# allenai/embodied-clip

Hardware: AMD Instinct MI355X
Metric: env-frames/sec (CLIP encode + policy fwd/bwd + PPO update) (higher is better)
Workload: dtype bf16

## Files before the change

embodied_clip_amd/csrc/conv_igemm.hip:

```cpp
#include <stdlib.h>

#include <algorithm>
#include <type_traits>
#include <utility>

#include "common.h"

thread_local int ec_tls_conv8_min_tiles = EC_CONV8_MIN_TILES_DEFAULT;

namespace {

inline int ec_tools_ablate() {
#ifdef EC_TOOLS
    static const int v = [] { const char* e = getenv("EC_CONV_ABLATE"); return e ? atoi(e) : 0; }();
    return v;
#else
    return 0;
#endif
}

constexpr int BK = 64;
constexpr int ROW_BYTES = BK * 2;

struct ConvArgs {
// ... 35 lines not shown

__device__ __forceinline__ float ec_relu(float x) { return __builtin_amdgcn_fmed3f(x, 0.f, __builtin_inff()); }
template <int ACT, bool RES, bool POOL, int FM, int FN, int PITCH>
__device__ __forceinline__ void epi_stage(const f32x16_t (&acc)[FM][FN], unsigned char* smem, const float* bias_n0,
                                          int row0, int col0, int lane) {
    const int frow = lane & 31, fhalf = lane >> 5;
#pragma unroll
    for (int j = 0; j < FN; ++j) {
        constexpr bool BIAS_UP_FRONT = !(RES && FM * FN <= 4);
        float4 bvj[4];
        if constexpr (BIAS_UP_FRONT) {
#pragma unroll
            for (int g = 0; g < 4; ++g)
                bvj[g] = bias_n0 ? *reinterpret_cast<const float4*>(bias_n0 + col0 + j * 32 + 8 * g + 4 * fhalf)
                                 : make_float4(0.f, 0.f, 0.f, 0.f);
        }
#pragma unroll
        for (int g = 0; g < 4; ++g) {
            if constexpr (!BIAS_UP_FRONT)
                bvj[g] = bias_n0 ? *reinterpret_cast<const float4*>(bias_n0 + col0 + j * 32 + 8 * g + 4 * fhalf)
                                 : make_float4(0.f, 0.f, 0.f, 0.f);
            const int lcol = col0 + j * 32 + 8 * g + 4 * fhalf;
            uint2 rr[FM];
            if constexpr (RES) {
#pragma unroll
                for (int i = 0; i < FM; ++i)
                    rr[i] = *reinterpret_cast<const uint2*>(smem + (row0 + i * 32 + frow) * PITCH + lcol * 2);
            }
#pragma unroll
            for (int i = 0; i < FM; ++i) {
                const int lrow_px = row0 + i * 32 + frow;
                float v0 = acc[i][j][4 * g + 0] + bvj[g].x, v1 = acc[i][j][4 * g + 1] + bvj[g].y;
                float v2 = acc[i][j][4 * g + 2] + bvj[g].z, v3 = acc[i][j][4 * g + 3] + bvj[g].w;
                if constexpr (POOL) {
                    v0 = ec_relu(v0); v1 = ec_relu(v1); v2 = ec_relu(v2); v3 = ec_relu(v3);
                    v0 += dpp_quad_xor1(v0); v1 += dpp_quad_xor1(v1); v2 += dpp_quad_xor1(v2); v3 += dpp_quad_xor1(v3);
                    v0 += dpp_quad_xor2(v0); v1 += dpp_quad_xor2(v1); v2 += dpp_quad_xor2(v2); v3 += dpp_quad_xor2(v3);
                    if ((lane & 3) == 0) {
                        uint2 o;
                        o.x = ec_pack2(0.25f * v0, 0.25f * v1);
                        o.y = ec_pack2(0.25f * v2, 0.25f * v3);
                        *reinterpret_cast<uint2*>(smem + (lrow_px >> 2) * PITCH + lcol * 2) = o;
                    }
                } else {
                    if constexpr (RES) {
                        v0 += ec_lo(rr[i].x); v1 += ec_hi(rr[i].x); v2 += ec_lo(rr[i].y); v3 += ec_hi(rr[i].y);
                    }
                    if constexpr (ACT == EC_ACT_RELU) {
                        v0 = ec_relu(v0); v1 = ec_relu(v1); v2 = ec_relu(v2); v3 = ec_relu(v3);
                    } else if constexpr (ACT == EC_ACT_QUICKGELU) {
                        v0 *= __builtin_amdgcn_rcpf(1.f + __expf(-1.702f * v0)); v1 *= __builtin_amdgcn_rcpf(1.f + __expf(-1.702f * v1));
                        v2 *= __builtin_amdgcn_rcpf(1.f + __expf(-1.702f * v2)); v3 *= __builtin_amdgcn_rcpf(1.f + __expf(-1.702f * v3));
                    }
                    uint2 o;
                    o.x = ec_pack2(v0, v1);
                    o.y = ec_pack2(v2, v3);
                    *reinterpret_cast<uint2*>(smem + lrow_px * PITCH + lcol * 2) = o;
                }
            }
        }
    }
}
template <bool POOL, bool RES_ONLY, int FM, int FN, int PITCH>
__device__ __forceinline__ void epi_stage_dispatch(const f32x16_t (&acc)[FM][FN], unsigned char* smem, const float* bias_n0,
                                                   int row0, int col0, int lane, int act, bool has_res) {
    if constexpr (POOL) {
        epi_stage<EC_ACT_RELU, false, true, FM, FN, PITCH>(acc, smem, bias_n0, row0, col0, lane);
    } else if constexpr (RES_ONLY) {
        if (act == EC_ACT_RELU) epi_stage<EC_ACT_RELU, true, false, FM, FN, PITCH>(acc, smem, bias_n0, row0, col0, lane);
        else epi_stage<EC_ACT_NONE, true, false, FM, FN, PITCH>(acc, smem, bias_n0, row0, col0, lane);
    } else {
        if (act == EC_ACT_RELU) {
            if (has_res) epi_stage<EC_ACT_RELU, true, false, FM, FN, PITCH>(acc, smem, bias_n0, row0, col0, lane);
            else epi_stage<EC_ACT_RELU, false, false, FM, FN, PITCH>(acc, smem, bias_n0, row0, col0, lane);
        } else if (act == EC_ACT_QUICKGELU) {
            epi_stage<EC_ACT_QUICKGELU, false, false, FM, FN, PITCH>(acc, smem, bias_n0, row0, col0, lane);
        } else {
            if (has_res) epi_stage<EC_ACT_NONE, true, false, FM, FN, PITCH>(acc, smem, bias_n0, row0, col0, lane);
            else epi_stage<EC_ACT_NONE, false, false, FM, FN, PITCH>(acc, smem, bias_n0, row0, col0, lane);
        }
    }
}

template <int ACT, int FM, int FN, int PITCH>
__device__ __forceinline__ void epi_stage_ln(const f32x16_t (&acc)[FM][FN], unsigned char* smem, const float* s_n0, const float* c_n0,
                                             const float2* rowab, int row0, int col0, int lane) {
    const int frow = lane & 31, fhalf = lane >> 5;
    float2 ab[FM];
#pragma unroll
    for (int i = 0; i < FM; ++i) ab[i] = rowab[row0 + i * 32 + frow];
#pragma unroll
    for (int j = 0; j < FN; ++j) {
        float4 sv[4], cv[4];
#pragma unroll
        for (int g = 0; g < 4; ++g) {
            sv[g] = *reinterpret_cast<const float4*>(s_n0 + col0 + j * 32 + 8 * g + 4 * fhalf);
            cv[g] = *reinterpret_cast<const float4*>(c_n0 + col0 + j * 32 + 8 * g + 4 * fhalf);
        }
#pragma unroll
        for (int g = 0; g < 4; ++g) {
            const int lcol = col0 + j * 32 + 8 * g + 4 * fhalf;
#pragma unroll
            for (int i = 0; i < FM; ++i) {
                const int lrow_px = row0 + i * 32 + frow;
                float v0 = fmaf(ab[i].x, acc[i][j][4 * g + 0], fmaf(ab[i].y, sv[g].x, cv[g].x));
                float v1 = fmaf(ab[i].x, acc[i][j][4 * g + 1], fmaf(ab[i].y, sv[g].y, cv[g].y));
                float v2 = fmaf(ab[i].x, acc[i][j][4 * g + 2], fmaf(ab[i].y, sv[g].z, cv[g].z));
                float v3 = fmaf(ab[i].x, acc[i][j][4 * g + 3], fmaf(ab[i].y, sv[g].w, cv[g].w));
                if constexpr (ACT == EC_ACT_QUICKGELU) {
                    v0 *= __builtin_amdgcn_rcpf(1.f + __expf(-1.702f * v0)); v1 *= __builtin_amdgcn_rcpf(1.f + __expf(-1.702f * v1));
                    v2 *= __builtin_amdgcn_rcpf(1.f + __expf(-1.702f * v2)); v3 *= __builtin_amdgcn_rcpf(1.f + __expf(-1.702f * v3));
                } else if constexpr (ACT == EC_ACT_RELU) {
                    v0 = ec_relu(v0); v1 = ec_relu(v1); v2 = ec_relu(v2); v3 = ec_relu(v3);
                }
                uint2 o;
                o.x = ec_pack2(v0, v1);
                o.y = ec_pack2(v2, v3);
                *reinterpret_cast<uint2*>(smem + lrow_px * PITCH + lcol * 2) = o;
            }
        }
    }
}

template <int R>
struct FragRing { u32x4_t f[R]; };
template <int I, int R, class AddrFn>
__device__ __forceinline__ void fr_issue(FragRing<R>& ring, AddrFn& addr) {
    asm volatile("ds_read_b128 %0, %1" : "=v"(ring.f[I % R]) : "v"(addr(std::integral_constant<int, I>{})));
}
template <int I, int R>
__device__ __forceinline__ void fr_tie(FragRing<R>& ring) { asm volatile("" : "+v"(ring.f[I % R])); }
template <int K, int NK, int G, int R, class AddrFn, class MmaFn>
__device__ __forceinline__ void fr_step(FragRing<R>& ring, AddrFn& addr, MmaFn& mma) {
    if constexpr (K < NK) {
        if constexpr (K + 1 < NK) {
            [&]<int... Q>(std::integer_sequence<int, Q...>) { (fr_issue<(K + 1) * G + Q, R>(ring, addr), ...); }
            (std::make_integer_sequence<int, G>{});
        }
        constexpr int after = (K + 1 < NK) ? G : 0;
        static_assert(G <= 15, "lgkmcnt is a 4-bit counter");
        asm volatile("s_waitcnt lgkmcnt(%0)" : : "n"(after));
        [&]<int... Q>(std::integer_sequence<int, Q...>) { (fr_tie<K * G + Q, R>(ring), ...); }(std::make_integer_sequence<int, G>{});
        mma(std::integral_constant<int, K>{}, ring);
        fr_step<K + 1, NK, G, R>(ring, addr, mma);
    }
}

template <int BM, int BN, int WM, int WN, int KS, bool POOL, bool PF, int MV, int NS, bool ILV = false, bool S2 = false>
__global__ __launch_bounds__(WM * WN * 64, (BM > 192) ? 2 : ((WM * WN == 8) ? 4 : (NS >= 3 ? 2 : 3))) void conv_igemm_kernel(ConvArgs p) {
    constexpr int TM = BM / WM, TN = BN / WN;
    constexpr int FM = TM / 32, FN = TN / 32;
    constexpr int NT = WM * WN * 64;
    constexpr int LR = NT / 8;
    constexpr int A_IT = BM / LR, B_IT = BN / LR;
    constexpr int A_BYTES = BM * ROW_BYTES, B_BYTES = BN * ROW_BYTES;
    static_assert(WM * WN == 4 || WM * WN == 8, "4 or 8 waves");
    static_assert(BM % LR == 0 && BN % LR == 0, "loader geometry");
    extern __shared__ __attribute__((aligned(16))) unsigned char smem[];

    const int tid = threadIdx.x;
    const int lane = tid & 63;
    const int wave = tid >> 6;
    const int wm = wave / WN, wn = wave % WN;

    const unsigned grid = gridDim.x;
    const unsigned lb = ec_xcd_remap(blockIdx.x, grid);
    static_assert(!ILV || (NS >= 3 && !PF && FM + FN <= 4), "interleaved pieces: ring mode with the inline-asm fragment stream");
    const int nvt = p.ntiles;
    int vt = (int)lb;
    if (vt >= nvt) return;
    int tile = vt;
    static_assert(MV <= BM && (MV == BM || !POOL), "padded tiles: non-pooled only");
    int m0 = (tile / p.ntn) * MV;
    int n0 = (tile % p.ntn) * BN;


    const int chunk = (tid & 7) ^ ((tid >> 4) & 7);
    const int lrow = tid >> 3;
    unsigned a_off[A_IT];
    unsigned a_msk[A_IT];
    unsigned b_off[B_IT];
    auto decode = [&]() {
#pragma unroll
        for (int i = 0; i < A_IT; ++i) {
            const int m = m0 + lrow + LR * i;
            int pix, y = 0, x = 0;
            if (POOL) {
                const int q = m >> 2, s2 = m & 3;
                const int Hp = p.H >> 1, Wp = p.W >> 1;
                const int b = q / (Hp * Wp);
                const int r2 = q - b * (Hp * Wp);
                const int yp = r2 / Wp;
                y = 2 * yp + (s2 >> 1);
                x = 2 * (r2 - yp * Wp) + (s2 & 1);
                pix = (b * p.H + y) * p.W + x;
            } else if (S2) {
                static_assert(!S2 || !POOL, "stride-2 instances have no fused pool");
                const int Ho = p.H >> 1, Wo = p.W >> 1;
                const int b = m / (Ho * Wo);
                const int r2 = m - b * (Ho * Wo);
                const int yo = r2 / Wo;
                y = 2 * yo;
// ... 201 lines not shown
                if (!(p.ablate & 2)) compute(cur);
                __syncthreads();
            }
        }
        }
        vt += (int)grid;
        const bool has_next = vt < nvt;
        if (has_next) {
            tile = vt;
            m0 = (tile / p.ntn) * MV;
            n0 = (tile % p.ntn) * BN;
            decode();
        }
        if (!(p.ablate & 8)) {
    if (has_res) {
        if (PREFETCH) {
#pragma unroll
            for (int i = 0; i < (PREFETCH ? NPASS : 1); ++i)
                *reinterpret_cast<uint4*>(smem + (i * RPP + srow) * PITCH + schunk * 16) = rres[i];
        } else {
#pragma unroll
            for (int i = 0; i < NPASS; ++i) {
                const int row = i * RPP + srow;
                uint4 v = make_uint4(0, 0, 0, 0);
#if defined(__HIP_DEVICE_COMPILE__)
                const unsigned off = (MV == BM || row < MV) ? ((unsigned)(orow0 + row) * (unsigned)p.Cout + (unsigned)(e_n0 + schunk * 8)) * 2u : 0xFFFFFFF0u;
                v = __builtin_bit_cast(uint4, __builtin_amdgcn_raw_buffer_load_b128(rs_res, (int)off, 0, 0));
#endif
                *reinterpret_cast<uint4*>(smem + row * PITCH + schunk * 16) = v;
            }
        }
        __syncthreads();
    }
    epi_stage_dispatch<POOL, PF, FM, FN, PITCH>(acc, smem, p.bias ? p.bias + e_n0 : nullptr, wm * TM, wn * TN, lane, p.act, has_res);
    __syncthreads();
#pragma unroll
    for (int r0 = 0; r0 < OUT_ROWS; r0 += RPP) {
        const int row = r0 + srow;
        if (orow0 + row < Mout && (MV == BM || row < MV))
            *reinterpret_cast<uint4*>(p.out + (long)(orow0 + row) * p.ldo + e_n0 + schunk * 8) =
                *reinterpret_cast<const uint4*>(smem + row * PITCH + schunk * 16);
    }
        }
        if (!has_next) break;
        __syncthreads();
    }
}

template <int BM, int BN, int WM, int WN, int KS, bool POOL, bool PF = false, int MV = BM, int NS = 0, bool ILV = false, bool S2 = false>
int launch(const ConvArgs& a, hipStream_t s) {
    ConvArgs p = a;
    p.ntn = a.Cout / BN;
    const int ntm = (a.M + MV - 1) / MV;
    p.ntiles = ntm * p.ntn;
    const size_t lds_max = 2 * (size_t)(BM + BN) * ROW_BYTES;
    const size_t epi = (size_t)(POOL ? BM / 4 : BM) * (BN * 2 + 16);
    p.nbuf = (BM * BN >= 256 * 256) ? 2 : 1;
    p.ablate = ec_tools_ablate();
    size_t lds = (size_t)(NS >= 3 ? NS : p.nbuf) * (BM + BN) * ROW_BYTES;
    if (lds < epi) lds = epi;
    auto kern = conv_igemm_kernel<BM, BN, WM, WN, KS, POOL, PF, MV, NS, ILV, S2>;
    static std::atomic<uint64_t> attr_done{0};
    if (auto attr_g_ = ec_attr_needed(attr_done)) {
        const size_t want = NS >= 3 ? lds : (lds_max > epi ? lds_max : epi);
        (void)hipFuncSetAttribute(reinterpret_cast<const void*>(kern), hipFuncAttributeMaxDynamicSharedMemorySize, (int)want);
    }
    const int wg_cap = 768;
    const int ring_per_cu = NS >= 3 ? (int)std::min<size_t>(2, (160 * 1024) / lds) : 0;
    const int cap = NS >= 3 ? 256 * ring_per_cu : ((BM * BN >= 256 * 256) ? 256 : wg_cap);
    const int nwg = p.ntiles < cap ? p.ntiles : cap;
    hipLaunchKernelGGL(kern, dim3((unsigned)nwg), dim3(WM * WN * 64), lds, s, p);
    EC_CHECK_LAUNCH();
    return EC_OK;
}


__device__ unsigned long long ec_dbg_stamps[2 * 1024];

template <int BN, int KS, bool POOL, int ABL, bool X3 = false, bool S2 = false, int BM = 256, int XP = 3>
__global__ __launch_bounds__(512, 2) void conv_igemm8_kernel(ConvArgs p) {
    static_assert(BM == 256 || (BM == 192 && BN == 128 && !POOL && !X3), "tile heights: 256; 192 for 128-wide 1x1 / 3x3 tiles");
    constexpr int WN = (BN >= 256 || BM == 192) ? 4 : 2, WMW = 8 / WN;
    constexpr int TM = BM / WMW, TN = BN / WN;
    constexpr int FM = TM / 32, FN = TN / 32;
    constexpr int NT = 512, LR = NT / 8;
    constexpr int A_IT = BM / LR, B_IT = BN / LR;
    constexpr int A_BYTES = BM * ROW_BYTES, B_BYTES = BN * ROW_BYTES, STAGE = A_BYTES + B_BYTES;
    static_assert(FN >= 1 && B_IT >= 1, "BN must be 128 or 256");
    constexpr bool LS = (ABL & 512) != 0 && BN == 128;
    extern __shared__ __attribute__((aligned(16))) unsigned char smem[];

    const unsigned long long t_entry = (ABL & 32) ? __builtin_amdgcn_s_memtime() : 0ull;
    const int tid = threadIdx.x;
    const int lane = tid & 63;
    const int wave = __builtin_amdgcn_readfirstlane(tid >> 6);
    const int wm = wave / WN, wn = wave % WN;
    const int grp = wave >> 2;

    const int tile = (int)ec_xcd_remap(blockIdx.x, gridDim.x);
    if (tile >= p.ntiles) return;
    const int m0 = (tile / p.ntn) * BM;
    const int n0 = (tile % p.ntn) * BN;

    constexpr bool LNOK = (KS == 1) && !POOL && !X3 && !S2;
    if constexpr (LNOK) {
        if (p.ln_stats && tid < BM) {
            float2 ab = make_float2(0.f, 0.f);
            const int row = m0 + tid;
            if (row < p.M) {
                const float4* rec = reinterpret_cast<const float4*>(p.ln_stats) + (size_t)row * p.ln_np;
                float4 r[8];
                float S = 0.f, Nn = 0.f;
#pragma unroll
                for (int q = 0; q < 8; ++q)
                    if (q < p.ln_np) { r[q] = rec[q]; S += r[q].x; Nn += r[q].z; }
                const float mean = S / Nn;
                float M2 = 0.f;
#pragma unroll
                for (int q = 0; q < 8; ++q)
                    if (q < p.ln_np) { const float d = r[q].x / r[q].z - mean; M2 += r[q].y + r[q].z * d * d; }
                const float rstd = rsqrtf(M2 / Nn + p.ln_eps);
                ab = make_float2(rstd, -mean * rstd);
            }
            reinterpret_cast<float2*>(smem + p.aux_off)[tid] = ab;
        }
    }

    const int chunk = (tid & 7) ^ ((tid >> 4) & 7);
    const int lrow = tid >> 3;
    unsigned a_off[A_IT], a_msk[A_IT], b_off[B_IT];
#pragma unroll
    for (int i = 0; i < A_IT; ++i) {
        const int m = m0 + lrow + LR * i;
        int pix, y = 0, x = 0;
        if (POOL) {
            const int q = m >> 2, s2 = m & 3;
            const int Hp = p.H >> 1, Wp = p.W >> 1;
            const int b = q / (Hp * Wp);
            const int r2 = q - b * (Hp * Wp);
            const int yp = r2 / Wp;
            y = 2 * yp + (s2 >> 1);
            x = 2 * (r2 - yp * Wp) + (s2 & 1);
            pix = (b * p.H + y) * p.W + x;
        } else if (S2) {
            static_assert(!S2 || !POOL, "stride-2 instances have no fused pool");
            const int Ho = p.H >> 1, Wo = p.W >> 1;
            const int b = m / (Ho * Wo);
            const int r2 = m - b * (Ho * Wo);
            const int yo = r2 / Wo;
            y = 2 * yo;
            x = 2 * (r2 - yo * Wo);
            pix = (b * p.H + y) * p.W + x;
        } else if (KS == 1) {
            pix = m;
        } else {
            const int b = m / (p.H * p.W);
            const int r2 = m - b * (p.H * p.W);
            y = r2 / p.W;
            x = r2 - y * p.W;
            pix = m;
        }
        unsigned msk = 1u;
        if (KS == 3) {
            const unsigned xm = (x > 0 ? 1u : 0u) | 2u | (x < p.W - 1 ? 4u : 0u);
            msk = (y > 0 ? xm : 0u) | (xm << 3) | (y < p.H - 1 ? (xm << 6) : 0u);
        }
        a_msk[i] = (m < p.M) ? msk : 0u;
        a_off[i] = (unsigned)pix * (unsigned)p.Cin * 2u + (unsigned)chunk * 16u;
    }
#pragma unroll
    for (int i = 0; i < B_IT; ++i) b_off[i] = ((unsigned)(n0 + lrow + LR * i) * (unsigned)(X3 ? 3 * p.K : p.K) + chunk * 8) * 2u;

#if defined(__HIP_DEVICE_COMPILE__)
    const __amdgpu_buffer_rsrc_t rs_in = __builtin_amdgcn_make_buffer_rsrc((void*)p.in, 0, p.in_bytes, 0x00020000);
    const __amdgpu_buffer_rsrc_t rs_w = __builtin_amdgcn_make_buffer_rsrc((void*)p.w, 0, p.w_bytes, 0x00020000);
#endif
    const int wave_lds = wave * 1024;
    const int nk = (X3 ? XP : 1) * (p.K / BK);

    int g_toff = 0; unsigned g_tapbit = 1u; int g_kb = 0;
    unsigned char* g_sa = smem; unsigned char* g_sb = smem; bool g_issue_a = true;
    auto glds_begin = [&](int kt, int buf) {
        g_sa = smem + buf * STAGE + wave_lds;
        g_sb = g_sa + A_BYTES;
        g_kb = kt * (BK * 2);
        g_toff = kt * (BK * 2);
        g_tapbit = 1u;
        if constexpr ((ABL & 64) != 0) g_issue_a = (kt % 9 == 0) || (kt % 9 == 4);
        if (X3) {
            const int ch = kt / XP, pl = (XP - 1) - (kt - XP * ch);
            g_toff = ch * (BK * 2);
            g_kb = (pl * p.K + ch * BK) * 2;
            g_sa = smem + (ch & 1) * A_BYTES + wave_lds;
            g_sb = smem + 2 * A_BYTES + (LS ? buf : (kt & 1)) * B_BYTES + wave_lds;
            g_issue_a = (kt == XP * ch);
        }
        if (KS == 3) {
            const int k = kt * BK;
            const int tap = k >> p.cin_log2, ci = k & (p.Cin - 1);
            const int ky = (tap * 11) >> 5;
            g_toff = (((ky - 1) * p.W + (tap - ky * 3 - 1)) * p.Cin + ci) * 2;
            g_tapbit = 1u << tap;
        }
    };
    auto glds_piece = [&](auto qc) {
        [[maybe_unused]] constexpr int q = decltype(qc)::value;
#if defined(__HIP_DEVICE_COMPILE__)
        if constexpr (q < A_IT) {
            if ((!X3 && !(ABL & 64)) || g_issue_a) {
                const unsigned off = (a_msk[q] & g_tapbit) ? a_off[q] + (unsigned)g_toff : 0xFFFFFFF0u;
                __builtin_amdgcn_raw_ptr_buffer_load_lds(rs_in, (lds_void_t*)(g_sa + q * (LR * ROW_BYTES)), 16, off, 0, 0, 0);
            }
        } else {
            constexpr int i = q - A_IT;
            __builtin_amdgcn_raw_ptr_buffer_load_lds(rs_w, (lds_void_t*)(g_sb + i * (LR * ROW_BYTES)), 16,
                                                     b_off[i] + (unsigned)g_kb, 0, 0, 0);
        }
#endif
    };

    f32x16_t acc[FM][FN];
#pragma unroll
    for (int i = 0; i < FM; ++i)
#pragma unroll
        for (int j = 0; j < FN; ++j)
#pragma unroll
            for (int r = 0; r < 16; ++r) acc[i][j][r] = 0.f;

    const int frow = lane & 31, fhalf = lane >> 5;
    constexpr bool DB = (ABL & 256) != 0 && !X3;
    unsigned bfo[FN];
#pragma unroll
    for (int j = 0; j < FN; ++j)
        bfo[j] = (unsigned)((n0 >> 5) + wn * (TN / 32) + j) * (unsigned)(p.K >> 4) * 1024u + (unsigned)lane * 16u;
#if defined(__HIP_DEVICE_COMPILE__)
    const __amdgpu_buffer_rsrc_t rs_wf = __builtin_amdgcn_make_buffer_rsrc((void*)p.w, 0, p.w_bytes, 0x00020000);
#endif
    s16x8_t fbd[2][2][FN];
    auto bload = [&](int kt, int h, int u) {
#if defined(__HIP_DEVICE_COMPILE__)
        const int soff = (kt * 4 + h * 2 + u) * 1024;
#pragma unroll
        for (int j = 0; j < FN; ++j)
            fbd[h][u][j] = __builtin_bit_cast(s16x8_t, __builtin_amdgcn_raw_buffer_load_b128(rs_wf, (int)bfo[j], soff, 0));
#endif
    };
    int fa_base[FM], fb_base[FN];
#pragma unroll
    for (int i = 0; i < FM; ++i) fa_base[i] = (wm * TM + i * 32 + frow) * ROW_BYTES;
#pragma unroll
    for (int j = 0; j < FN; ++j) fb_base[j] = A_BYTES + (wn * TN + j * 32 + frow) * ROW_BYTES;
    const int fsw = (frow >> 1) & 7;

    s16x8_t fa[LS ? 4 : 2][FM], fb[LS ? 4 : 2][FN];
    auto read_half = [&](int kt, int stg, auto hc) {
        constexpr int h = decltype(hc)::value;
        constexpr int fo = LS ? 2 * h : 0;
        const unsigned char* sta = smem + stg * STAGE;
        const unsigned char* stb = sta;
        if (X3) {
            sta = smem + ((kt / XP) & 1) * A_BYTES;
            stb = smem + A_BYTES + stg * B_BYTES;
        }
#pragma unroll
        for (int u = 0; u < 2; ++u) {
            const int c = ((h * 2 + u) * 2 + fhalf) ^ fsw;
#pragma unroll
            for (int i = 0; i < FM; ++i) fa[fo + u][i] = *reinterpret_cast<const s16x8_t*>(sta + fa_base[i] + (c << 4));
            if constexpr (!DB) {
#pragma unroll
                for (int j = 0; j < FN; ++j) fb[fo + u][j] = *reinterpret_cast<const s16x8_t*>(stb + fb_base[j] + (c << 4));
            }
        }
    };
    using I0 = std::integral_constant<int, 0>;
    using I1 = std::integral_constant<int, 1>;

    constexpr int NPIECE = DB ? A_IT : A_IT + B_IT;
    glds_begin(0, 0);
    [&]<int... Q>(std::integer_sequence<int, Q...>) { (glds_piece(std::integral_constant<int, Q>{}), ...); }
    (std::make_integer_sequence<int, NPIECE>{});
    asm volatile("s_waitcnt vmcnt(0)" ::: "memory");
    __builtin_amdgcn_s_barrier();
    if constexpr (DB) { bload(0, 0, 0); bload(0, 0, 1); bload(0, 1, 0); bload(0, 1, 1); }
    auto issue_all = [&](int kt, int buf) {
        glds_begin(kt, buf);
        [&]<int... Q>(std::integer_sequence<int, Q...>) { (glds_piece(std::integral_constant<int, Q>{}), ...); }
        (std::make_integer_sequence<int, NPIECE>{});
    };
    unsigned poff[A_IT + B_IT];
    auto prep = [&](int kt, int buf) {
        glds_begin(kt, buf);
#pragma unroll
        for (int q = 0; q < A_IT; ++q) poff[q] = (a_msk[q] & g_tapbit) ? a_off[q] + (unsigned)g_toff : 0xFFFFFFF0u;
        if constexpr (!DB) {
#pragma unroll
            for (int i = 0; i < B_IT; ++i) poff[A_IT + i] = b_off[i] + (unsigned)g_kb;
        }
    };
    auto piece_pre = [&](auto qc) {
        [[maybe_unused]] constexpr int q = decltype(qc)::value;
#if defined(__HIP_DEVICE_COMPILE__)
        if constexpr (q < A_IT) {
            if ((!X3 && !(ABL & 64)) || g_issue_a)
                __builtin_amdgcn_raw_ptr_buffer_load_lds(rs_in, (lds_void_t*)(g_sa + q * (LR * ROW_BYTES)), 16, poff[q], 0, 0, 0);
        } else {
            __builtin_amdgcn_raw_ptr_buffer_load_lds(rs_w, (lds_void_t*)(g_sb + (q - A_IT) * (LR * ROW_BYTES)), 16, poff[q], 0, 0, 0);
        }
#endif
    };
    auto mfma16 = [&](auto issue_c, auto hc, int kt) {
        constexpr bool ISSUE = decltype(issue_c)::value;
        [[maybe_unused]] constexpr int H = decltype(hc)::value;
        constexpr int fo = LS ? 2 * H : 0;
        constexpr int PN = LS ? (NPIECE + 1 - H) / 2 : NPIECE, PBASE = LS ? (H ? (NPIECE + 1) / 2 : 0) : 0;
        [&]<int... Q>(std::integer_sequence<int, Q...>) {
            ([&] {
                constexpr int u = Q / (FM * FN), r = Q % (FM * FN), i = r / FN, j = r % FN;
                if constexpr (!(ABL & 2))
                    acc[i][j] = __builtin_amdgcn_mfma_f32_32x32x16_bf16(
                        __builtin_bit_cast(bf16x8_t, DB ? fbd[H][u][j] : fb[fo + u][j]), __builtin_bit_cast(bf16x8_t, fa[fo + u][i]), acc[i][j], 0, 0, 0);
                if constexpr (DB && r == FM * FN - 1) {
                    bload(kt + 1, H, u);
                    __builtin_amdgcn_sched_barrier(0);
                }
                constexpr int NP = PN, EVERY = (2 * FM * FN) / (NP > 0 ? NP : 1);
                if constexpr (ISSUE && NP > 0 && Q % EVERY == EVERY - 1 && Q / EVERY < NP) {
                    piece_pre(std::integral_constant<int, PBASE + Q / EVERY>{});
                    __builtin_amdgcn_sched_barrier(0);
                }
            }(), ...);
        }(std::make_integer_sequence<int, 2 * FM * FN>{});
    };
    using BT = std::true_type;
    using BF = std::false_type;
    if constexpr (LS) {
        if (nk > 1) issue_all(1, 1);
        if (grp) __builtin_amdgcn_s_barrier();
    } else
    if (grp) {
        if (nk > 1 && !(ABL & 1)) issue_all(1, 1);
        if constexpr (!(ABL & 16)) __builtin_amdgcn_s_barrier();
    }

    constexpr int abl = ABL;
    const bool dbg = (abl & 32) && blockIdx.x == 0 && (wave == 0 || wave == 4) && lane == 0;
    unsigned long long* dbg_lds = reinterpret_cast<unsigned long long*>(smem + 2 * STAGE) + grp * 256;
    int dbg_i = 0;
    auto stamp = [&]() { if constexpr ((abl & 32) != 0) if (dbg && dbg_i < 256) dbg_lds[dbg_i++] = __builtin_amdgcn_s_memtime(); };
    auto ktile = [&](int kt, auto gc, auto ic) {
        constexpr int G = decltype(gc)::value;
        constexpr bool ISSUE = decltype(ic)::value;
        const int cur = kt & 1;
        if constexpr (!(abl & 4)) read_half(kt, cur, I0{});
        if constexpr (G == 0 && ISSUE) prep(kt + 1, cur ^ 1);
        asm volatile("s_waitcnt lgkmcnt(0)" ::: "memory");
        __builtin_amdgcn_sched_barrier(0);
        stamp();
        if constexpr (!(abl & 16)) __builtin_amdgcn_s_barrier();
        stamp();
        __builtin_amdgcn_s_setprio(1);
        mfma16(std::bool_constant<(G == 0 && ISSUE)>{}, I0{}, kt);
        __builtin_amdgcn_s_setprio(0);
        __builtin_amdgcn_sched_barrier(0);
        stamp();
        if constexpr (!(abl & 16)) __builtin_amdgcn_s_barrier();
        stamp();
        if constexpr (!(abl & 4)) read_half(kt, cur, I1{});
        if constexpr (G == 1 && ISSUE) prep(kt + 2, cur);
        asm volatile("s_waitcnt lgkmcnt(0)" ::: "memory");
        if constexpr (G == 1) { if constexpr (DB) asm volatile("s_waitcnt vmcnt(%0)" : : "n"(2 * FN) : "memory"); else asm volatile("s_waitcnt vmcnt(0)" ::: "memory"); }
        __builtin_amdgcn_sched_barrier(0);
        stamp();
        if constexpr (!(abl & 16)) __builtin_amdgcn_s_barrier();
        stamp();
        __builtin_amdgcn_s_setprio(1);
        mfma16(std::bool_constant<(G == 1 && ISSUE)>{}, I1{}, kt);
        __builtin_amdgcn_s_setprio(0);
        if constexpr (G == 0) { if constexpr (DB) asm volatile("s_waitcnt vmcnt(%0)" : : "n"(2 * FN) : "memory"); else asm volatile("s_waitcnt vmcnt(0)" ::: "memory"); }
        __builtin_amdgcn_sched_barrier(0);
        stamp();
        if constexpr (!(abl & 16)) __builtin_amdgcn_s_barrier();
        stamp();
    };
    auto kloop = [&](auto gc) {
        constexpr int G = decltype(gc)::value;
        const int n_issue = (abl & 1) ? 0 : nk - 1 - G;
        int kt = 0;
        for (; kt < n_issue; ++kt) ktile(kt, gc, BT{});
        for (; kt < nk; ++kt) ktile(kt, gc, BF{});
    };
    auto ktile_ls = [&](int kt, int stg, int stg2, auto ic) {
        constexpr bool ISSUE = decltype(ic)::value;
        read_half(kt, stg, I0{});
        read_half(kt, stg, I1{});
        if constexpr (ISSUE) prep(kt + 2, stg2);
        asm volatile("s_waitcnt lgkmcnt(0)" ::: "memory");
        asm volatile("s_waitcnt vmcnt(0)" ::: "memory");
        __builtin_amdgcn_sched_barrier(0);
        __builtin_amdgcn_s_barrier();
        __builtin_amdgcn_s_setprio(1);
        mfma16(std::bool_constant<ISSUE>{}, I0{}, kt);
        mfma16(std::bool_constant<ISSUE>{}, I1{}, kt);
        __builtin_amdgcn_s_setprio(0);
        __builtin_amdgcn_sched_barrier(0);
        __builtin_amdgcn_s_barrier();
    };
    if constexpr (LS) {
        int stg = 0, stg2 = 2, kt = 0;
        for (; kt < nk - 2; ++kt) {
            ktile_ls(kt, stg, stg2, BT{});
            stg = (stg == 2) ? 0 : stg + 1;
            stg2 = (stg2 == 2) ? 0 : stg2 + 1;
        }
        for (; kt < nk; ++kt) {
            ktile_ls(kt, stg, stg2, BF{});
            stg = (stg == 2) ? 0 : stg + 1;
        }
        if (!grp) __builtin_amdgcn_s_barrier();
    } else {
    if (grp) kloop(I1{}); else kloop(I0{});
    if (!grp && !(ABL & 16)) __builtin_amdgcn_s_barrier();
    }
    __syncthreads();
    const unsigned long long t_loop_end = (ABL & 32) ? __builtin_amdgcn_s_memtime() : 0ull;
    if constexpr ((abl & 32) != 0) if (dbg) {
        for (int i = 0; i < 256; ++i) ec_dbg_stamps[grp * 1024 + i] = i < dbg_i ? dbg_lds[i] : 0ull;
        ec_dbg_stamps[grp * 1024 + 300] = t_entry;
        ec_dbg_stamps[grp * 1024 + 301] = t_loop_end;
    }
    if constexpr ((abl & 32) != 0) __syncthreads();

    if constexpr (X3) {
        static_assert(!X3 || (BN == 128 && !POOL && KS == 1), "X3: 128-wide 1x1 tiles");
        constexpr int PITCHF = BN * 4 + 16;
        float* outf = reinterpret_cast<float*>(p.out);
#pragma unroll
        for (int pass = 0; pass < 2; ++pass) {
            if ((wm >> 1) == pass) {
#pragma unroll
                for (int j = 0; j < FN; ++j)
#pragma unroll
                    for (int g = 0; g < 4; ++g) {
                        const int lcol = wn * TN + j * 32 + 8 * g + 4 * fhalf;
                        float4 bv = make_float4(0.f, 0.f, 0.f, 0.f);
                        if (p.bias) bv = *reinterpret_cast<const float4*>(p.bias + n0 + lcol);
#pragma unroll
                        for (int i = 0; i < FM; ++i) {
                            const int lr = (wm & 1) * TM + i * 32 + frow;
                            float4 v = make_float4(acc[i][j][4 * g + 0] + bv.x, acc[i][j][4 * g + 1] + bv.y,
                                                   acc[i][j][4 * g + 2] + bv.z, acc[i][j][4 * g + 3] + bv.w);
                            if (p.act == EC_ACT_RELU) {
                                v.x = fmaxf(v.x, 0.f); v.y = fmaxf(v.y, 0.f); v.z = fmaxf(v.z, 0.f); v.w = fmaxf(v.w, 0.f);
                            }
                            *reinterpret_cast<float4*>(smem + lr * PITCHF + lcol * 4) = v;
                        }
                    }
            }
            __syncthreads();
#pragma unroll
            for (int r0 = 0; r0 < 128; r0 += NT / 32) {
                const int row = r0 + (tid >> 5), ch = tid & 31;
                const long grow = (long)m0 + pass * 128 + row;
                if (grow < p.M)
                    *reinterpret_cast<float4*>(outf + grow * p.Cout + n0 + ch * 4) =
                        *reinterpret_cast<const float4*>(smem + row * PITCHF + ch * 16);
            }
            __syncthreads();
        }
        return;
    }
    if constexpr ((ABL & 8) != 0) return;
    constexpr int CH = BN / 8;
    constexpr int PITCH = BN * 2 + 16;
    constexpr int RPP = NT / CH;
    constexpr int OUT_ROWS = POOL ? BM / 4 : BM;
    constexpr int NPASS = OUT_ROWS / RPP;
    const int Mout = POOL ? (p.M >> 2) : p.M;
    const int orow0 = POOL ? (m0 >> 2) : m0;
    const int srow = tid / CH, schunk = tid % CH;
    const bool has_res = !POOL && (p.res != nullptr);
#if defined(__HIP_DEVICE_COMPILE__)
    const __amdgpu_buffer_rsrc_t rs_res8 = __builtin_amdgcn_make_buffer_rsrc((void*)p.res, 0, p.res ? p.res_bytes : 0u, 0x00020000);
#endif
    if (has_res) {
#pragma unroll
        for (int i = 0; i < NPASS; ++i) {
            const int row = i * RPP + srow;
            uint4 v = make_uint4(0, 0, 0, 0);
#if defined(__HIP_DEVICE_COMPILE__)
            const unsigned off = ((unsigned)(orow0 + row) * (unsigned)p.Cout + (unsigned)(n0 + schunk * 8)) * 2u;
            v = __builtin_bit_cast(uint4, __builtin_amdgcn_raw_buffer_load_b128(rs_res8, (int)off, 0, 0));
#endif
            *reinterpret_cast<uint4*>(smem + row * PITCH + schunk * 16) = v;
        }
        __syncthreads();
    }
    bool ln_done = false;
    if constexpr (LNOK) {
        if (p.ln_stats) {
            const float2* rowab = reinterpret_cast<const float2*>(smem + p.aux_off);
            if (p.act == EC_ACT_QUICKGELU) epi_stage_ln<EC_ACT_QUICKGELU, FM, FN, PITCH>(acc, smem, p.ln_s + n0, p.bias + n0, rowab, wm * TM, wn * TN, lane);
            else epi_stage_ln<EC_ACT_NONE, FM, FN, PITCH>(acc, smem, p.ln_s + n0, p.bias + n0, rowab, wm * TM, wn * TN, lane);
            ln_done = true;
        }
    }
    if (!ln_done)
    epi_stage_dispatch<POOL, false, FM, FN, PITCH>(acc, smem, p.bias ? p.bias + n0 : nullptr, wm * TM, wn * TN, lane, p.act, has_res);
    __syncthreads();
#pragma unroll
    for (int r0 = 0; r0 < OUT_ROWS; r0 += RPP) {
        const int row = r0 + srow;
        const uint4 v = *reinterpret_cast<const uint4*>(smem + row * PITCH + schunk * 16);
        if (orow0 + row < Mout && !(ABL & 128))
            *reinterpret_cast<uint4*>(p.out + (long)(orow0 + row) * p.ldo + n0 + schunk * 8) = v;
        if constexpr (LNOK) {
            if (p.stats_out) {
                float x[8] = {ec_lo(v.x), ec_hi(v.x), ec_lo(v.y), ec_hi(v.y), ec_lo(v.z), ec_hi(v.z), ec_lo(v.w), ec_hi(v.w)};
                float sm = ((x[0] + x[1]) + (x[2] + x[3])) + ((x[4] + x[5]) + (x[6] + x[7]));
#pragma unroll
                for (int o = CH / 2; o > 0; o >>= 1) sm += __shfl_xor(sm, o, 64);
                const float mu = sm * (1.f / (float)BN);
                float q = 0.f;
#pragma unroll
                for (int e = 0; e < 8; ++e) { const float d = x[e] - mu; q = fmaf(d, d, q); }
#pragma unroll
                for (int o = CH / 2; o > 0; o >>= 1) q += __shfl_xor(q, o, 64);
                if (schunk == 0 && orow0 + row < Mout)
                    reinterpret_cast<float4*>(p.stats_out)[(size_t)(orow0 + row) * p.ntn + (tile % p.ntn)] = make_float4(sm, q, (float)BN, 0.f);
            }
        }
    }
    if constexpr ((ABL & 32) != 0) if (blockIdx.x == 0 && (wave == 0 || wave == 4) && lane == 0) ec_dbg_stamps[grp * 1024 + 302] = __builtin_amdgcn_s_memtime();
}

template <int BN, int KS, bool POOL, bool X3 = false, bool S2 = false, int BM = 256, int XP = 3>
int launch8(const ConvArgs& a, hipStream_t s) {
    ConvArgs p = a;
    p.ntn = a.Cout / BN;
    p.ntiles = ((a.M + BM - 1) / BM) * p.ntn;
// ... 286 lines not shown
```

Baseline: 64120.

## Switch 8-wave conv igemm from 32x32x16 to 16x16x32 bf16 MFMA fragments

Rewrites the 8-wave implicit-GEMM conv kernel to use 16x16x32 bf16 MFMA tiles instead of 32x32x16. Fragment bookkeeping, LDS read addressing, direct B-weight prefetch offsets, the vmcnt waits and all epilogues (bias/residual/pool, LN, fp32 X3) change to the 4-element accumulator layout. The aim is fewer LDS fragment reads per k-step and lower register pressure, but it issues more MFMA instructions. It also requires the pre-packed weight layout to match the new 16-column, 32-k blocking, and it adds realtime debug stamps.

```diff
diff --git a/embodied_clip_amd/csrc/conv_igemm.hip b/embodied_clip_amd/csrc/conv_igemm.hip
--- a/embodied_clip_amd/csrc/conv_igemm.hip
+++ b/embodied_clip_amd/csrc/conv_igemm.hip
@@ -141,42 +141,100 @@
     }
 }
 
-template <int ACT, int FM, int FN, int PITCH>
-__device__ __forceinline__ void epi_stage_ln(const f32x16_t (&acc)[FM][FN], unsigned char* smem, const float* s_n0, const float* c_n0,
-                                             const float2* rowab, int row0, int col0, int lane) {
-    const int frow = lane & 31, fhalf = lane >> 5;
-    float2 ab[FM];
-#pragma unroll
-    for (int i = 0; i < FM; ++i) ab[i] = rowab[row0 + i * 32 + frow];
+template <int ACT, bool RES, bool POOL, int FM, int FN, int PITCH>
+__device__ __forceinline__ void epi_stage(const f32x4_t (&acc)[FM][FN], unsigned char* smem, const float* bias_n0,
+                                          int row0, int col0, int lane) {
+    const int frow = lane & 15, fq = lane >> 4;
+    float4 bv[FN];
+#pragma unroll
+    for (int j = 0; j < FN; ++j)
+        bv[j] = bias_n0 ? *reinterpret_cast<const float4*>(bias_n0 + col0 + j * 16 + 4 * fq) : make_float4(0.f, 0.f, 0.f, 0.f);
 #pragma unroll
     for (int j = 0; j < FN; ++j) {
-        float4 sv[4], cv[4];
-#pragma unroll
-        for (int g = 0; g < 4; ++g) {
-            sv[g] = *reinterpret_cast<const float4*>(s_n0 + col0 + j * 32 + 8 * g + 4 * fhalf);
-            cv[g] = *reinterpret_cast<const float4*>(c_n0 + col0 + j * 32 + 8 * g + 4 * fhalf);
-        }
-#pragma unroll
-        for (int g = 0; g < 4; ++g) {
-            const int lcol = col0 + j * 32 + 8 * g + 4 * fhalf;
-#pragma unroll
-            for (int i = 0; i < FM; ++i) {
-                const int lrow_px = row0 + i * 32 + frow;
-                float v0 = fmaf(ab[i].x, acc[i][j][4 * g + 0], fmaf(ab[i].y, sv[g].x, cv[g].x));
-                float v1 = fmaf(ab[i].x, acc[i][j][4 * g + 1], fmaf(ab[i].y, sv[g].y, cv[g].y));
-                float v2 = fmaf(ab[i].x, acc[i][j][4 * g + 2], fmaf(ab[i].y, sv[g].z, cv[g].z));
-                float v3 = fmaf(ab[i].x, acc[i][j][4 * g + 3], fmaf(ab[i].y, sv[g].w, cv[g].w));
-                if constexpr (ACT == EC_ACT_QUICKGELU) {
+        const int lcol = col0 + j * 16 + 4 * fq;
+        uint2 rr[FM];
+        if constexpr (RES) {
+#pragma unroll
+            for (int i = 0; i < FM; ++i)
+                rr[i] = *reinterpret_cast<const uint2*>(smem + (row0 + i * 16 + frow) * PITCH + lcol * 2);
+        }
+#pragma unroll
+        for (int i = 0; i < FM; ++i) {
+            const int lrow_px = row0 + i * 16 + frow;
+            float v0 = acc[i][j][0] + bv[j].x, v1 = acc[i][j][1] + bv[j].y;
+            float v2 = acc[i][j][2] + bv[j].z, v3 = acc[i][j][3] + bv[j].w;
+            if constexpr (POOL) {
+                v0 = ec_relu(v0); v1 = ec_relu(v1); v2 = ec_relu(v2); v3 = ec_relu(v3);
+                v0 += dpp_quad_xor1(v0); v1 += dpp_quad_xor1(v1); v2 += dpp_quad_xor1(v2); v3 += dpp_quad_xor1(v3);
+                v0 += dpp_quad_xor2(v0); v1 += dpp_quad_xor2(v1); v2 += dpp_quad_xor2(v2); v3 += dpp_quad_xor2(v3);
+                if ((lane & 3) == 0) {
+                    uint2 o;
+                    o.x = ec_pack2(0.25f * v0, 0.25f * v1);
+                    o.y = ec_pack2(0.25f * v2, 0.25f * v3);
+                    *reinterpret_cast<uint2*>(smem + (lrow_px >> 2) * PITCH + lcol * 2) = o;
+                }
+            } else {
+                if constexpr (RES) {
+                    v0 += ec_lo(rr[i].x); v1 += ec_hi(rr[i].x); v2 += ec_lo(rr[i].y); v3 += ec_hi(rr[i].y);
+                }
+                if constexpr (ACT == EC_ACT_RELU) {
+                    v0 = ec_relu(v0); v1 = ec_relu(v1); v2 = ec_relu(v2); v3 = ec_relu(v3);
+                } else if constexpr (ACT == EC_ACT_QUICKGELU) {
                     v0 *= __builtin_amdgcn_rcpf(1.f + __expf(-1.702f * v0)); v1 *= __builtin_amdgcn_rcpf(1.f + __expf(-1.702f * v1));
                     v2 *= __builtin_amdgcn_rcpf(1.f + __expf(-1.702f * v2)); v3 *= __builtin_amdgcn_rcpf(1.f + __expf(-1.702f * v3));
-                } else if constexpr (ACT == EC_ACT_RELU) {
-                    v0 = ec_relu(v0); v1 = ec_relu(v1); v2 = ec_relu(v2); v3 = ec_relu(v3);
                 }
                 uint2 o;
                 o.x = ec_pack2(v0, v1);
                 o.y = ec_pack2(v2, v3);
                 *reinterpret_cast<uint2*>(smem + lrow_px * PITCH + lcol * 2) = o;
             }
+        }
+    }
+}
+template <bool POOL, bool RES_ONLY, int FM, int FN, int PITCH>
+__device__ __forceinline__ void epi_stage_dispatch(const f32x4_t (&acc)[FM][FN], unsigned char* smem, const float* bias_n0,
+                                                   int row0, int col0, int lane, int act, bool has_res) {
+    static_assert(!RES_ONLY, "the 8-wave kernel carries every variant");
+    if constexpr (POOL) {
+        epi_stage<EC_ACT_RELU, false, true, FM, FN, PITCH>(acc, smem, bias_n0, row0, col0, lane);
+    } else if (act == EC_ACT_RELU) {
+        if (has_res) epi_stage<EC_ACT_RELU, true, false, FM, FN, PITCH>(acc, smem, bias_n0, row0, col0, lane);
+        else epi_stage<EC_ACT_RELU, false, false, FM, FN, PITCH>(acc, smem, bias_n0, row0, col0, lane);
+    } else if (act == EC_ACT_QUICKGELU) {
+        epi_stage<EC_ACT_QUICKGELU, false, false, FM, FN, PITCH>(acc, smem, bias_n0, row0, col0, lane);
+    } else {
+        if (has_res) epi_stage<EC_ACT_NONE, true, false, FM, FN, PITCH>(acc, smem, bias_n0, row0, col0, lane);
+        else epi_stage<EC_ACT_NONE, false, false, FM, FN, PITCH>(acc, smem, bias_n0, row0, col0, lane);
+    }
+}
+template <int ACT, int FM, int FN, int PITCH>
+__device__ __forceinline__ void epi_stage_ln(const f32x4_t (&acc)[FM][FN], unsigned char* smem, const float* s_n0, const float* c_n0,
+                                             const float2* rowab, int row0, int col0, int lane) {
+    const int frow = lane & 15, fq = lane >> 4;
+    float2 ab[FM];
+#pragma unroll
+    for (int i = 0; i < FM; ++i) ab[i] = rowab[row0 + i * 16 + frow];
+#pragma unroll
+    for (int j = 0; j < FN; ++j) {
+        const int lcol = col0 + j * 16 + 4 * fq;
+        const float4 sv = *reinterpret_cast<const float4*>(s_n0 + lcol), cv = *reinterpret_cast<const float4*>(c_n0 + lcol);
+#pragma unroll
+        for (int i = 0; i < FM; ++i) {
+            const int lrow_px = row0 + i * 16 + frow;
+            float v0 = fmaf(ab[i].x, acc[i][j][0], fmaf(ab[i].y, sv.x, cv.x));
+            float v1 = fmaf(ab[i].x, acc[i][j][1], fmaf(ab[i].y, sv.y, cv.y));
+            float v2 = fmaf(ab[i].x, acc[i][j][2], fmaf(ab[i].y, sv.z, cv.z));
+            float v3 = fmaf(ab[i].x, acc[i][j][3], fmaf(ab[i].y, sv.w, cv.w));
+            if constexpr (ACT == EC_ACT_QUICKGELU) {
+                v0 *= __builtin_amdgcn_rcpf(1.f + __expf(-1.702f * v0)); v1 *= __builtin_amdgcn_rcpf(1.f + __expf(-1.702f * v1));
+                v2 *= __builtin_amdgcn_rcpf(1.f + __expf(-1.702f * v2)); v3 *= __builtin_amdgcn_rcpf(1.f + __expf(-1.702f * v3));
+            } else if constexpr (ACT == EC_ACT_RELU) {
+                v0 = ec_relu(v0); v1 = ec_relu(v1); v2 = ec_relu(v2); v3 = ec_relu(v3);
+            }
+            uint2 o;
+            o.x = ec_pack2(v0, v1);
+            o.y = ec_pack2(v2, v3);
+            *reinterpret_cast<uint2*>(smem + lrow_px * PITCH + lcol * 2) = o;
         }
     }
 }
@@ -544,7 +602,7 @@
     static_assert(BM == 256 || (BM == 192 && BN == 128 && !POOL && !X3), "tile heights: 256; 192 for 128-wide 1x1 / 3x3 tiles");
     constexpr int WN = (BN >= 256 || BM == 192) ? 4 : 2, WMW = 8 / WN;
     constexpr int TM = BM / WMW, TN = BN / WN;
-    constexpr int FM = TM / 32, FN = TN / 32;
+    constexpr int FM = TM / 16, FN = TN / 16;
     constexpr int NT = 512, LR = NT / 8;
     constexpr int A_IT = BM / LR, B_IT = BN / LR;
     constexpr int A_BYTES = BM * ROW_BYTES, B_BYTES = BN * ROW_BYTES, STAGE = A_BYTES + B_BYTES;
@@ -553,6 +611,7 @@
     extern __shared__ __attribute__((aligned(16))) unsigned char smem[];
 
     const unsigned long long t_entry = (ABL & 32) ? __builtin_amdgcn_s_memtime() : 0ull;
+    const unsigned long long r_entry = (ABL & 32) ? __builtin_amdgcn_s_memrealtime() : 0ull;
     const int tid = threadIdx.x;
     const int lane = tid & 63;
     const int wave = __builtin_amdgcn_readfirstlane(tid >> 6);
@@ -681,58 +740,51 @@
 #endif
     };
 
-    f32x16_t acc[FM][FN];
+    f32x4_t acc[FM][FN];
 #pragma unroll
     for (int i = 0; i < FM; ++i)
 #pragma unroll
         for (int j = 0; j < FN; ++j)
 #pragma unroll
-            for (int r = 0; r < 16; ++r) acc[i][j][r] = 0.f;
-
-    const int frow = lane & 31, fhalf = lane >> 5;
+            for (int r = 0; r < 4; ++r) acc[i][j][r] = 0.f;
+
+    const int frow = lane & 15, fq = lane >> 4;
     constexpr bool DB = (ABL & 256) != 0 && !X3;
     unsigned bfo[FN];
 #pragma unroll
     for (int j = 0; j < FN; ++j)
-        bfo[j] = (unsigned)((n0 >> 5) + wn * (TN / 32) + j) * (unsigned)(p.K >> 4) * 1024u + (unsigned)lane * 16u;
+        bfo[j] = (unsigned)((n0 >> 4) + wn * (TN / 16) + j) * (unsigned)(p.K >> 5) * 1024u + (unsigned)lane * 16u;
 #if defined(__HIP_DEVICE_COMPILE__)
     const __amdgpu_buffer_rsrc_t rs_wf = __builtin_amdgcn_make_buffer_rsrc((void*)p.w, 0, p.w_bytes, 0x00020000);
 #endif
-    s16x8_t fbd[2][2][FN];
-    auto bload = [&](int kt, int h, int u) {
+    s16x8_t fbd[2][FN];
+    auto bload = [&](int kt, int h) {
 #if defined(__HIP_DEVICE_COMPILE__)
-        const int soff = (kt * 4 + h * 2 + u) * 1024;
+        const int soff = (kt * 2 + h) * 1024;
 #pragma unroll
         for (int j = 0; j < FN; ++j)
-            fbd[h][u][j] = __builtin_bit_cast(s16x8_t, __builtin_amdgcn_raw_buffer_load_b128(rs_wf, (int)bfo[j], soff, 0));
+            fbd[h][j] = __builtin_bit_cast(s16x8_t, __builtin_amdgcn_raw_buffer_load_b128(rs_wf, (int)bfo[j], soff, 0));
 #endif
     };
-    int fa_base[FM], fb_base[FN];
-#pragma unroll
-    for (int i = 0; i < FM; ++i) fa_base[i] = (wm * TM + i * 32 + frow) * ROW_BYTES;
-#pragma unroll
-    for (int j = 0; j < FN; ++j) fb_base[j] = A_BYTES + (wn * TN + j * 32 + frow) * ROW_BYTES;
+    const int fa_base = (wm * TM + frow) * ROW_BYTES, fb_base = A_BYTES + (wn * TN + frow) * ROW_BYTES;
     const int fsw = (frow >> 1) & 7;
 
-    s16x8_t fa[LS ? 4 : 2][FM], fb[LS ? 4 : 2][FN];
+    s16x8_t fa[LS ? 2 : 1][FM], fb[LS ? 2 : 1][FN];
     auto read_half = [&](int kt, int stg, auto hc) {
         constexpr int h = decltype(hc)::value;
-        constexpr int fo = LS ? 2 * h : 0;
+        constexpr int fo = LS ? h : 0;
         const unsigned char* sta = smem + stg * STAGE;
         const unsigned char* stb = sta;
         if (X3) {
             sta = smem + ((kt / XP) & 1) * A_BYTES;
             stb = smem + A_BYTES + stg * B_BYTES;
         }
-#pragma unroll
-        for (int u = 0; u < 2; ++u) {
-            const int c = ((h * 2 + u) * 2 + fhalf) ^ fsw;
-#pragma unroll
-            for (int i = 0; i < FM; ++i) fa[fo + u][i] = *reinterpret_cast<const s16x8_t*>(sta + fa_base[i] + (c << 4));
-            if constexpr (!DB) {
-#pragma unroll
-                for (int j = 0; j < FN; ++j) fb[fo + u][j] = *reinterpret_cast<const s16x8_t*>(stb + fb_base[j] + (c << 4));
-            }
+        const int c = (h * 4 + fq) ^ fsw;
+#pragma unroll
+        for (int i = 0; i < FM; ++i) fa[fo][i] = *reinterpret_cast<const s16x8_t*>(sta + fa_base + (c << 4) + i * (16 * ROW_BYTES));
+        if constexpr (!DB) {
+#pragma unroll
+            for (int j = 0; j < FN; ++j) fb[fo][j] = *reinterpret_cast<const s16x8_t*>(stb + fb_base + (c << 4) + j * (16 * ROW_BYTES));
         }
     };
     using I0 = std::integral_constant<int, 0>;
@@ -744,7 +796,7 @@
     (std::make_integer_sequence<int, NPIECE>{});
     asm volatile("s_waitcnt vmcnt(0)" ::: "memory");
     __builtin_amdgcn_s_barrier();
-    if constexpr (DB) { bload(0, 0, 0); bload(0, 0, 1); bload(0, 1, 0); bload(0, 1, 1); }
+    if constexpr (DB) { bload(0, 0); bload(0, 1); }
     auto issue_all = [&](int kt, int buf) {
         glds_begin(kt, buf);
         [&]<int... Q>(std::integer_sequence<int, Q...>) { (glds_piece(std::integral_constant<int, Q>{}), ...); }
@@ -774,25 +826,25 @@
     auto mfma16 = [&](auto issue_c, auto hc, int kt) {
         constexpr bool ISSUE = decltype(issue_c)::value;
         [[maybe_unused]] constexpr int H = decltype(hc)::value;
-        constexpr int fo = LS ? 2 * H : 0;
+        constexpr int fo = LS ? H : 0;
         constexpr int PN = LS ? (NPIECE + 1 - H) / 2 : NPIECE, PBASE = LS ? (H ? (NPIECE + 1) / 2 : 0) : 0;
         [&]<int... Q>(std::integer_sequence<int, Q...>) {
             ([&] {
-                constexpr int u = Q / (FM * FN), r = Q % (FM * FN), i = r / FN, j = r % FN;
+                constexpr int i = Q / FN, j = Q % FN;
                 if constexpr (!(ABL & 2))
-                    acc[i][j] = __builtin_amdgcn_mfma_f32_32x32x16_bf16(
-                        __builtin_bit_cast(bf16x8_t, DB ? fbd[H][u][j] : fb[fo + u][j]), __builtin_bit_cast(bf16x8_t, fa[fo + u][i]), acc[i][j], 0, 0, 0);
-                if constexpr (DB && r == FM * FN - 1) {
-                    bload(kt + 1, H, u);
+                    acc[i][j] = __builtin_amdgcn_mfma_f32_16x16x32_bf16(
+                        __builtin_bit_cast(bf16x8_t, DB ? fbd[H][j] : fb[fo][j]), __builtin_bit_cast(bf16x8_t, fa[fo][i]), acc[i][j], 0, 0, 0);
+                if constexpr (DB && Q == FM * FN - 1) {
+                    bload(kt + 1, H);
                     __builtin_amdgcn_sched_barrier(0);
                 }
-                constexpr int NP = PN, EVERY = (2 * FM * FN) / (NP > 0 ? NP : 1);
+                constexpr int NP = PN, EVERY = (FM * FN) / (NP > 0 ? NP : 1);
                 if constexpr (ISSUE && NP > 0 && Q % EVERY == EVERY - 1 && Q / EVERY < NP) {
                     piece_pre(std::integral_constant<int, PBASE + Q / EVERY>{});
                     __builtin_amdgcn_sched_barrier(0);
                 }
             }(), ...);
-        }(std::make_integer_sequence<int, 2 * FM * FN>{});
+        }(std::make_integer_sequence<int, FM * FN>{});
     };
     using BT = std::true_type;
     using BF = std::false_type;
@@ -831,7 +883,7 @@
         if constexpr (!(abl & 4)) read_half(kt, cur, I1{});
         if constexpr (G == 1 && ISSUE) prep(kt + 2, cur);
         asm volatile("s_waitcnt lgkmcnt(0)" ::: "memory");
-        if constexpr (G == 1) { if constexpr (DB) asm volatile("s_waitcnt vmcnt(%0)" : : "n"(2 * FN) : "memory"); else asm volatile("s_waitcnt vmcnt(0)" ::: "memory"); }
+        if constexpr (G == 1) { if constexpr (DB) asm volatile("s_waitcnt vmcnt(%0)" : : "n"(FN) : "memory"); else asm volatile("s_waitcnt vmcnt(0)" ::: "memory"); }
         __builtin_amdgcn_sched_barrier(0);
         stamp();
         if constexpr (!(abl & 16)) __builtin_amdgcn_s_barrier();
@@ -839,7 +891,7 @@
         __builtin_amdgcn_s_setprio(1);
         mfma16(std::bool_constant<(G == 1 && ISSUE)>{}, I1{}, kt);
         __builtin_amdgcn_s_setprio(0);
-        if constexpr (G == 0) { if constexpr (DB) asm volatile("s_waitcnt vmcnt(%0)" : : "n"(2 * FN) : "memory"); else asm volatile("s_waitcnt vmcnt(0)" ::: "memory"); }
+        if constexpr (G == 0) { if constexpr (DB) asm volatile("s_waitcnt vmcnt(%0)" : : "n"(FN) : "memory"); else asm volatile("s_waitcnt vmcnt(0)" ::: "memory"); }
         __builtin_amdgcn_sched_barrier(0);
         stamp();
         if constexpr (!(abl & 16)) __builtin_amdgcn_s_barrier();
@@ -886,10 +938,13 @@
     }
     __syncthreads();
     const unsigned long long t_loop_end = (ABL & 32) ? __builtin_amdgcn_s_memtime() : 0ull;
+    const unsigned long long r_loop_end = (ABL & 32) ? __builtin_amdgcn_s_memrealtime() : 0ull;
     if constexpr ((abl & 32) != 0) if (dbg) {
         for (int i = 0; i < 256; ++i) ec_dbg_stamps[grp * 1024 + i] = i < dbg_i ? dbg_lds[i] : 0ull;
         ec_dbg_stamps[grp * 1024 + 300] = t_entry;
         ec_dbg_stamps[grp * 1024 + 301] = t_loop_end;
+        ec_dbg_stamps[grp * 1024 + 303] = r_entry;
+        ec_dbg_stamps[grp * 1024 + 304] = r_loop_end;
     }
     if constexpr ((abl & 32) != 0) __syncthreads();
 
@@ -901,23 +956,20 @@
         for (int pass = 0; pass < 2; ++pass) {
             if ((wm >> 1) == pass) {
 #pragma unroll
-                for (int j = 0; j < FN; ++j)
-#pragma unroll
-                    for (int g = 0; g < 4; ++g) {
-                        const int lcol = wn * TN + j * 32 + 8 * g + 4 * fhalf;
-                        float4 bv = make_float4(0.f, 0.f, 0.f, 0.f);
-                        if (p.bias) bv = *reinterpret_cast<const float4*>(p.bias + n0 + lcol);
-#pragma unroll
-                        for (int i = 0; i < FM; ++i) {
-                            const int lr = (wm & 1) * TM + i * 32 + frow;
-                            float4 v = make_float4(acc[i][j][4 * g + 0] + bv.x, acc[i][j][4 * g + 1] + bv.y,
-                                                   acc[i][j][4 * g + 2] + bv.z, acc[i][j][4 * g + 3] + bv.w);
-                            if (p.act == EC_ACT_RELU) {
-                                v.x = fmaxf(v.x, 0.f); v.y = fmaxf(v.y, 0.f); v.z = fmaxf(v.z, 0.f); v.w = fmaxf(v.w, 0.f);
-                            }
-                            *reinterpret_cast<float4*>(smem + lr * PITCHF + lcol * 4) = v;
+                for (int j = 0; j < FN; ++j) {
+                    const int lcol = wn * TN + j * 16 + 4 * fq;
+                    float4 bv = make_float4(0.f, 0.f, 0.f, 0.f);
+                    if (p.bias) bv = *reinterpret_cast<const float4*>(p.bias + n0 + lcol);
+#pragma unroll
+                    for (int i = 0; i < FM; ++i) {
+                        const int lr = (wm & 1) * TM + i * 16 + frow;
+                        float4 v = make_float4(acc[i][j][0] + bv.x, acc[i][j][1] + bv.y, acc[i][j][2] + bv.z, acc[i][j][3] + bv.w);
+                        if (p.act == EC_ACT_RELU) {
+                            v.x = fmaxf(v.x, 0.f); v.y = fmaxf(v.y, 0.f); v.z = fmaxf(v.z, 0.f); v.w = fmaxf(v.w, 0.f);
                         }
+                        *reinterpret_cast<float4*>(smem + lr * PITCHF + lcol * 4) = v;
                     }
+                }
             }
             __syncthreads();
 #pragma unroll
```

Result: no change. 64670 (median of 6 runs) (+0.9%).
